# prime-slam/octreelib

Hardware: NVIDIA B200
Metric: points/sec (insert+subdivide+per-leaf RANSAC) (higher is better)
Workload: dtype f64

## Files before the change

octreelib_b200/csrc/common.cuh:

```cuda
#pragma once
#include <cuda_runtime.h>
#include <math.h>
#include <stdint.h>
#include <stdio.h>
#include <stdlib.h>
#include <string.h>

#include <algorithm>
#include <iterator>
#include <map>
#include <mutex>
#include <string>
#include <vector>

#include "../../include/octreelib_b200.h"

namespace ol {

struct Error {
    int code;
    std::string msg;
};

void set_last_error(int code, const std::string& msg);
// ... 316 lines not shown
    void raw_free(void* p) {
        if (g_block_cache.put(cache_key(), p)) return;
        if (free_fn)
            free_fn(alloc_user, p);
        else
            cudaFreeAsync(p, stream);
    }
    void sync() { OL_CUDA(cudaStreamSynchronize(stream)); }

    static constexpr size_t STATUS_POOL_WORDS = (size_t)1 << 20;
    unsigned long long* status_pool = nullptr;
    size_t status_used = 0;
    unsigned long long* status_words(size_t words) {
        words = (words + 1) & ~(size_t)1;
        if (status_used + words > STATUS_POOL_WORDS) return nullptr;
        if (!status_pool) {
            status_pool = static_cast<unsigned long long*>(alloc(STATUS_POOL_WORDS * 8));
            OL_CUDA(cudaMemsetAsync(status_pool, 0, STATUS_POOL_WORDS * 8, stream));
        }
        unsigned long long* p = status_pool + status_used;
        status_used += words;
        return p;
    }
    ~Ctx() {
        if (status_pool) free(status_pool, STATUS_POOL_WORDS * 8);
        trim_pool();
        release_arena();
    }
};

struct PoolScope {
    Ctx& c;
    explicit PoolScope(Ctx& ctx) : c(ctx) { c.pool_enabled = true; }
    ~PoolScope() {
        c.pool_enabled = false;
        c.trim_pool();
    }
};

struct ProfScope {
    Ctx& c;
    Profiler::Rec rec{};
    bool on;
    ProfScope(Ctx& ctx, const char* name, double units = 0.0) : c(ctx), on(ctx.prof && ctx.prof->enabled) {
        if (on) {
            rec.name = name;
            rec.units = units;
            rec.a = c.prof->get_event();
            rec.b = c.prof->get_event();
            cudaEventRecord(rec.a, c.stream);
        }
    }
    ~ProfScope() {
        if (on) {
            cudaEventRecord(rec.b, c.stream);
            c.prof->recs.push_back(rec);
        }
    }
};

struct Mail {
    volatile unsigned long long* slot = nullptr;
    unsigned long long ticket = 0;
    const uint32_t* err = nullptr;
    const uint32_t* aux = nullptr;
};
struct MailResult {
    unsigned long long total = 0;
    uint32_t err = 0, aux = 0;
};
#ifdef __CUDACC__
__device__ __forceinline__ void mail_post(const Mail& m, unsigned long long total) {
    if (!m.slot) return;
    m.slot[1] = total;
    m.slot[2] = m.err ? (unsigned long long)*reinterpret_cast<const volatile uint32_t*>(m.err) : 0ull;
    m.slot[3] = m.aux ? (unsigned long long)*reinterpret_cast<const volatile uint32_t*>(m.aux) : 0ull;
    __threadfence_system();
    m.slot[0] = m.ticket;
}
#endif
extern unsigned long long g_mail_ticket;
MailResult mail_wait(const Mail& m, cudaStream_t stream);

template <typename T>
struct DevBuf {
    Ctx* ctx = nullptr;
    T* ptr = nullptr;
    size_t count = 0;

    DevBuf() = default;
    DevBuf(Ctx& c, size_t n) { reset(c, n); }
    DevBuf(const DevBuf&) = delete;
    DevBuf& operator=(const DevBuf&) = delete;
    DevBuf(DevBuf&& o) noexcept { *this = std::move(o); }
    DevBuf& operator=(DevBuf&& o) noexcept {
        if (this != &o) {
            release();
            ctx = o.ctx;
            ptr = o.ptr;
            count = o.count;
            o.ptr = nullptr;
            o.count = 0;
        }
        return *this;
    }
    ~DevBuf() { release(); }
    void reset(Ctx& c, size_t n) {
        release();
        ctx = &c;
        count = n;
        ptr = static_cast<T*>(c.alloc(n * sizeof(T)));
    }
    void release() {
        if (ptr && ctx) ctx->free(ptr, count * sizeof(T));
        ptr = nullptr;
        count = 0;
    }
    void swap(DevBuf& o) {
        std::swap(ctx, o.ctx);
        std::swap(ptr, o.ptr);
        std::swap(count, o.count);
    }
    void zero() {
        if (count) OL_CUDA(cudaMemsetAsync(ptr, 0, count * sizeof(T), ctx->stream));
    }
    T* get() const { return ptr; }
    size_t size() const { return count; }
};

template <typename T>
inline void d2h(Ctx& c, T* host, const T* dev, size_t n) {
    if (n) OL_CUDA(cudaMemcpyAsync(host, dev, n * sizeof(T), cudaMemcpyDeviceToHost, c.stream));
}
template <typename T>
inline void h2d(Ctx& c, T* dev, const T* host, size_t n) {
    if (n) OL_CUDA(cudaMemcpyAsync(dev, host, n * sizeof(T), cudaMemcpyHostToDevice, c.stream));
}
template <typename T>
inline void d2d(Ctx& c, T* dst, const T* src, size_t n) {
    if (n) OL_CUDA(cudaMemcpyAsync(dst, src, n * sizeof(T), cudaMemcpyDeviceToDevice, c.stream));
}

inline unsigned grid_for(size_t n, int threads) { return (unsigned)((n + threads - 1) / threads); }

__host__ __device__ inline double npy_floor_divide_ref(double a, double b) {
    if (b == 0.0) return a / b;
    double mod = fmod(a, b);
    double div = (a - mod) / b;
    if (mod != 0.0) {
        if ((b < 0) != (mod < 0)) {
            div -= 1.0;
        }
    }
    double floordiv;
    if (div != 0.0) {
        floordiv = floor(div);
        if (div - floordiv > 0.5) floordiv += 1.0;
    } else {
        floordiv = copysign(0.0, a / b);
    }
    return floordiv;
}

__host__ __device__ inline double npy_floor_divide(double a, double b) {
    if (!(b > 0.0) || !(fabs(a) < 1.7e308) || !(b < 1.7e308)) return npy_floor_divide_ref(a, b);
    double q = floor(a / b);
// ... 40 lines not shown
```

octreelib_b200/csrc/forest.cu:

```cuda
#include <algorithm>
#include <climits>
#include <exception>
#include <mutex>

#include "forest.cuh"
#include "primitives.cuh"

namespace ol {

__device__ __forceinline__ int seg_of_rank(const uint32_t* __restrict__ seg_start, int n_seg, uint32_t r) {
    const uint32_t total = seg_start[n_seg];
    int s = (int)((float)r * __fdividef((float)n_seg, (float)(total ? total : 1u)));
    s = s < 0 ? 0 : (s >= n_seg ? n_seg - 1 : s);
    int lo = 0, hi = n_seg;
#pragma unroll 1
    for (int probe = 0; probe < 3; ++probe) {
        if (seg_start[s] > r) {
            hi = s;
            s = s - 1;
        } else if (seg_start[s + 1] <= r) {
            lo = s + 1;
            s = s + 1;
        } else {
            return s;
// ... 145 lines not shown
                qa = 0.0;
            }
            q[a] = (long long)qa;
            long long rel = q[a] - kp.qmin[a];
            if (rel < 0) {
                e |= DEVERR_CELL_RANGE;
                rel = 0;
            }
            if (kp.shift[a] < 64) key |= ((uint64_t)rel) << kp.shift[a];
        }
    }
    if (kp.pose_bits) key |= (uint64_t)seg_pose[seg_of_rank(seg_start, n_seg, r)];
    double c[3];
#pragma unroll
    for (int a = 0; a < 3; ++a) c[a] = cell_corner_coord(q[a], kp.corner[a], kp.edge, kp.single_cell);
    int bad;
    MortT m = (MortT)point_morton(p, c, kp.edge, kp.depth, &bad);
    if (embed_levels > 0) {
        key = (key << (3 * embed_levels + 1)) | ((uint64_t)(bad < kp.depth ? 1u : 0u) << (3 * embed_levels)) | (uint64_t)m;
    } else {
        if (bad < kp.depth) m |= MortBits<MortT>::bad;
        mort[r] = m;
    }
    keys[r] = (KeyT)key;
    vals[r] = r;
    if (e) atomicOr(err, e);
}

template <typename MortT>
__global__ void __launch_bounds__(256) remorton_kernel(const double* __restrict__ xyz, const uint32_t* __restrict__ perm,
                                                       const uint32_t* __restrict__ cell_of, const uint32_t* __restrict__ lcell,
                                                       const uint64_t* __restrict__ cell_key, KeyParams kp, uint32_t n,
                                                       MortT* __restrict__ mort) {
    uint32_t i = blockIdx.x * blockDim.x + threadIdx.x;
    if (i >= n) return;
    const size_t r = perm[i];
    uint32_t c = cell_of[i];
    if (lcell) c = lcell[c];
    long long q[3] = {0, 0, 0};
    if (!kp.single_cell) unpack_cell(kp, cell_key[c], q);
    const double p[3] = {xyz[r * 3], xyz[r * 3 + 1], xyz[r * 3 + 2]};
    double c0[3];
#pragma unroll
    for (int a = 0; a < 3; ++a) c0[a] = cell_corner_coord(q[a], kp.corner[a], kp.edge, kp.single_cell);
    int bad;
    MortT m = (MortT)point_morton(p, c0, kp.edge, kp.depth, &bad);
    if (bad < kp.depth) m |= MortBits<MortT>::bad;
    mort[i] = m;
}

template <typename KeyT>
struct CellKeyFn {
    const KeyT* keys;
    int pose_bits;
    __device__ uint64_t operator()(uint32_t i) const { return (uint64_t)(keys[i] >> pose_bits); }
};
template <typename KeyT>
struct CellKeyEmbedFn {
    const KeyT* keys;
    int shift;
    int fw;
    uint32_t* mort_out;
    __device__ uint64_t operator()(uint32_t i) const {
        const KeyT k = keys[i];
        const uint32_t field = (uint32_t)k & ((1u << fw) - 1u);
        mort_out[i] = (field & ((1u << (fw - 1)) - 1u)) | ((field >> (fw - 1)) ? MortBits<uint32_t>::bad : 0u);
        return (uint64_t)(k >> shift);
    }
};
struct CellEmitFn {
    uint64_t* cell_key;
    uint32_t* cell_start;
    __device__ void operator()(uint32_t run, uint32_t i, uint64_t key) const {
        cell_key[run] = key;
        cell_start[run] = i;
    }
};
struct GroupPoseKeyFn {
    const uint32_t* group;
    const uint32_t* perm;
    const uint32_t* seg_start;
    const int32_t* seg_pose;
    int n_seg;
    __device__ uint64_t operator()(uint32_t i) const {
        return ((uint64_t)group[i] << 32) | (uint64_t)(uint32_t)seg_pose[seg_of_rank(seg_start, n_seg, perm[i])];
    }
};
struct CellPoseEmitFn {
    uint32_t* cp_cell;
    int32_t* cp_pose;
    int32_t* cell_first_pose;
    const uint32_t* cellidx;
    __device__ void operator()(uint32_t run, uint32_t i, uint64_t key) const {
        const uint32_t cell = (uint32_t)(key >> 32);
        cp_cell[run] = cell;
        cp_pose[run] = (int32_t)(uint32_t)key;
        if (i == 0 || cellidx[i - 1] != cell) cell_first_pose[cell] = (int32_t)(uint32_t)key;
    }
};
struct BlockEmitFn {
    uint32_t* blk_start;
    uint32_t* blk_leaf;
    int32_t* blk_pose;
    __device__ void operator()(uint32_t run, uint32_t i, uint64_t key) const {
        blk_start[run] = i;
        blk_leaf[run] = (uint32_t)(key >> 32);
        blk_pose[run] = (int32_t)(uint32_t)key;
    }
};

constexpr int CMP_THREADS = 256;
constexpr int CMP_TILE = 2048;
constexpr int CMP_WORDS = CMP_TILE / 32;

__global__ void __launch_bounds__(CMP_THREADS) keep_bits_kernel(const uint8_t* __restrict__ keep, const uint32_t* __restrict__ via,
                                                                uint32_t n, uint32_t* __restrict__ bits,
                                                                uint32_t* __restrict__ tile_cnt) {
    __shared__ uint32_t s_cnt;
    if (threadIdx.x == 0) s_cnt = 0;
    __syncthreads();
    const uint32_t base = blockIdx.x * CMP_TILE;
    const int lane = threadIdx.x & 31;
    uint32_t c = 0;
    uint8_t flag[CMP_TILE / CMP_THREADS];
#pragma unroll
    for (int j = 0; j < CMP_TILE / CMP_THREADS; ++j) {
        const uint32_t i = base + j * CMP_THREADS + threadIdx.x;
        flag[j] = i < n ? keep[via ? via[i] : i] : (uint8_t)0;
    }
#pragma unroll
    for (int j = 0; j < CMP_TILE / CMP_THREADS; ++j) {
        const uint32_t i = base + j * CMP_THREADS + threadIdx.x;
        const bool k = flag[j] != 0;
        const uint32_t m = __ballot_sync(0xffffffffu, k);
        if (lane == 0 && i < n) {
            bits[i >> 5] = m;
            c += __popc(m);
        }
    }
    if (lane == 0 && c) atomicAdd(&s_cnt, c);
    __syncthreads();
    if (threadIdx.x == 0) tile_cnt[blockIdx.x] = s_cnt;
}

template <typename MortT>
__global__ void __launch_bounds__(CMP_THREADS) compact_move_kernel(const uint32_t* __restrict__ bits, const uint32_t* __restrict__ tile_off,
                                                                   uint32_t n, const uint32_t* __restrict__ perm_in,
                                                                   const MortT* __restrict__ mort_in, const uint32_t* __restrict__ aux_in,
                                                                   uint32_t* __restrict__ perm_out, MortT* __restrict__ mort_out,
                                                                   uint32_t* __restrict__ aux_out, uint32_t* __restrict__ word_off) {
    __shared__ uint32_t s_mask[CMP_WORDS], s_off[CMP_WORDS], s_half;
    const uint32_t base = blockIdx.x * CMP_TILE;
    const uint32_t n_words = (n + 31) >> 5;
    const int lane = threadIdx.x & 31, warp = threadIdx.x >> 5;
    if (threadIdx.x < CMP_WORDS) {
        const uint32_t w = (base >> 5) + threadIdx.x;
        const uint32_t m = w < n_words ? bits[w] : 0u;
        const uint32_t c = __popc(m);
        uint32_t inc = c;
#pragma unroll
        for (int d = 1; d < 32; d <<= 1) {
            const uint32_t v = __shfl_up_sync(0xffffffffu, inc, d);
            if (lane >= d) inc += v;
        }
        if (threadIdx.x == 31) s_half = inc;
        s_mask[threadIdx.x] = m;
        s_off[threadIdx.x] = inc - c;
    }
    __syncthreads();
// ... 548 lines not shown
__global__ void cell_first_leaf_kernel(uint32_t L, const uint32_t* __restrict__ lcell, uint32_t* __restrict__ cell_leaf_begin) {
    uint32_t k = blockIdx.x * blockDim.x + threadIdx.x;
    if (k >= L) return;
    const uint32_t c = lcell[k];
    if (k == 0 || lcell[k - 1] != c) cell_leaf_begin[c] = k;
}

__global__ void leaf_order_geometry_kernel(uint32_t L, const uint32_t* __restrict__ lcell, const int32_t* __restrict__ lparent,
                                           const uint8_t* __restrict__ lchild, const uint64_t* __restrict__ lpath,
                                           const uint8_t* __restrict__ ldepth, const uint32_t* __restrict__ irank,
                                           const uint32_t* __restrict__ imask, const uint32_t* __restrict__ leafbase,
                                           const uint32_t* __restrict__ cell_ifirst, const uint32_t* __restrict__ cell_leaf_begin,
                                           const uint64_t* __restrict__ cell_key, KeyParams kp, uint32_t* __restrict__ cache_rank,
                                           uint32_t* __restrict__ leaf_by_cache, double* __restrict__ corner,
                                           double* __restrict__ edge) {
    uint32_t k = blockIdx.x * blockDim.x + threadIdx.x;
    if (k >= L) return;
    const uint32_t c = lcell[k];
    uint32_t j = cell_leaf_begin[c];
    const int32_t p = lparent[k];
    if (p >= 0) {
        const uint32_t ch = lchild[k];
        j += leafbase[irank[p]] - leafbase[cell_ifirst[c]] + (uint32_t)__popc(~imask[p] & ((1u << ch) - 1u));
    }
    cache_rank[k] = j;
    leaf_by_cache[j] = k;
    long long q[3] = {0, 0, 0};
    if (!kp.single_cell) unpack_cell(kp, cell_key[c], q);
    double co[3];
    for (int a = 0; a < 3; ++a) co[a] = cell_corner_coord(q[a], kp.corner[a], kp.edge, kp.single_cell);
    double e = kp.edge;
    const int depth = ldepth[k];
    const uint64_t path = lpath[k];
    for (int d = 0; d < depth; ++d) {
        const double h = e * 0.5;
        const uint32_t dig = (uint32_t)(path >> (3 * (depth - 1 - d))) & 7u;
        if (dig & 4u) co[0] = co[0] + h;
        if (dig & 2u) co[1] = co[1] + h;
        if (dig & 1u) co[2] = co[2] + h;
        e = h;
    }
    corner[(size_t)j * 3 + 0] = co[0];
    corner[(size_t)j * 3 + 1] = co[1];
    corner[(size_t)j * 3 + 2] = co[2];
    edge[j] = e;
}

__global__ void __launch_bounds__(256) block_max_kernel(const uint32_t* __restrict__ blk_start, const unsigned long long* __restrict__ d_nb,
                                                        uint32_t* __restrict__ out_max) {
    __shared__ uint32_t s_w[8];
    const uint32_t nb = (uint32_t)*d_nb;
    uint32_t v = 0;
    for (uint32_t b = blockIdx.x * blockDim.x + threadIdx.x; b < nb; b += gridDim.x * blockDim.x) {
        const uint32_t sz = blk_start[b + 1] - blk_start[b];
        v = sz > v ? sz : v;
    }
#pragma unroll
    for (int o = 16; o > 0; o >>= 1) {
        uint32_t t = __shfl_xor_sync(0xffffffffu, v, o);
        v = t > v ? t : v;
    }
    if ((threadIdx.x & 31) == 0) s_w[threadIdx.x >> 5] = v;
    __syncthreads();
    if (threadIdx.x == 0) {
        for (int w = 1; w < 8; ++w) v = s_w[w] > v ? s_w[w] : v;
        if (v) atomicMax(out_max, v);
    }
}

__global__ void block_keep_kernel(uint32_t nb, const uint32_t* __restrict__ blk_start, const int32_t* __restrict__ blk_pose,
                                  const uint8_t* __restrict__ listed, const uint8_t* __restrict__ table,
                                  long long table_len, uint8_t* __restrict__ keep_blk) {
    uint32_t b = blockIdx.x * blockDim.x + threadIdx.x;
    if (b >= nb) return;
    uint8_t keep = 1;
    if (!listed || listed[blk_pose[b]]) {
        long long sz = (long long)(blk_start[b + 1] - blk_start[b]);
        if (sz > table_len - 1) sz = table_len - 1;
        keep = table[sz];
    }
    keep_blk[b] = keep;
}

__global__ void pos_keep_from_block_kernel(uint32_t n, const uint32_t* __restrict__ blk_of_pos,
                                           const uint8_t* __restrict__ keep_blk, uint8_t* __restrict__ keep_pos) {
    uint32_t i = blockIdx.x * blockDim.x + threadIdx.x;
    if (i < n) keep_pos[i] = keep_blk[blk_of_pos[i]];
}

}

#include "forest_host.inl"
#include "forest_host2.inl"
```

octreelib_b200/csrc/forest.cuh:

```cuda
#pragma once
#include <initializer_list>
#include <vector>

#include "common.cuh"
#include "pointkey.cuh"

namespace ol {

constexpr int MORTON_INITIAL_DEPTH = 8;
constexpr int MORTON32_MAX_DEPTH = 10;

struct Forest {
    Ctx ctx;
    ol_forest_config cfg{};
    int max_depth = OL_MAX_DEPTH;

    DevBuf<double> P64;
    size_t cap = 0, N = 0;
    size_t bbox_done = 0;
    bool q_known = false;
    long long q_lo[3] = {0, 0, 0}, q_hi[3] = {0, 0, 0};
    bool points_external() const { return P64.ptr != nullptr && P64.ctx == nullptr; }
    void adopt_points(double* ext, size_t n, const int64_t* seg_sizes, const int32_t* seg_pose_in, const int64_t* seg_first_in,
                      int n_segments, int n_poses_total, const long long qlo[3], const long long qhi[3]);
// ... 25 lines not shown
    bool cells_pending = false, blocks_pending = false;
    Mail cells_mail{}, blocks_mail{};
    DevBuf<unsigned long long> d_nb;
    void resolve_cells();
    void resolve_blocks();
    void resolve_pending() {
        resolve_cells();
        resolve_blocks();
    }
    void build_enqueue();
    void ensure_blocks_enqueue();
    void prefetch_tables();

    bool built = false;
    KeyParams kp{};
    int key_bits = 0;
    int key_embed = 0;
    uint32_t A0 = 0;
    DevBuf<uint32_t> perm0;
    DevBuf<uint64_t> mort0;
    bool mort32 = true;
    size_t mort_len(size_t n) const { return mort32 ? (n + 1) / 2 : n; }
    DevBuf<uint32_t> cellidx0;
    uint32_t C = 0;
    DevBuf<uint64_t> cell_key;
    DevBuf<uint32_t> cell_start0;
    uint32_t CP = 0;
    bool cp_valid = false;
    DevBuf<uint32_t> cp_cell;
    DevBuf<int32_t> cp_pose;
    DevBuf<int32_t> cell_first_pose;

    bool shaped = false;
    bool order_virgin = false;
    uint32_t A = 0;
    uint32_t A_shape = 0;
    DevBuf<uint32_t> perm;
    DevBuf<uint64_t> mort;
    DevBuf<uint32_t> leaf_of;
    uint32_t L = 0;
    DevBuf<uint32_t> lstart;
    DevBuf<uint32_t> lcell;
    DevBuf<int32_t> lparent;
    DevBuf<uint64_t> lpath;
    DevBuf<uint8_t> ldepth;
    DevBuf<uint8_t> lchild;
    uint32_t I = 0;
    size_t icap = 0;
    DevBuf<uint32_t> istart;
    DevBuf<uint32_t> icell;
    DevBuf<uint8_t> idepth;
    DevBuf<uint64_t> ipath;
    DevBuf<int32_t> iparent;
    DevBuf<uint8_t> ichild;
    std::vector<uint32_t> level_ibegin;
    int depth_reached = 0;

    bool order_valid = false;
    DevBuf<uint32_t> cache_rank;
    DevBuf<uint32_t> leaf_by_cache;
    DevBuf<double> leaf_corner;
    DevBuf<double> leaf_edge;
    DevBuf<uint32_t> cell_leaf_begin;

    bool replay_pending = false;
    uint32_t sp_n = 0;
    DevBuf<long long> sp_q;
    DevBuf<uint32_t> sp_depth;
    DevBuf<uint64_t> sp_path;
    DevBuf<uint32_t> sp_epoch;

    int n_subdivide_calls = 0;
    std::vector<int> pose_epoch;
    bool epochs_valid = false;
    DevBuf<uint32_t> iepoch;
    bool history_active() const { return n_subdivide_calls >= 2 && epochs_valid && I > 0; }
    void assign_epochs(int epoch, const uint64_t* sorted_keys, const uint32_t* sorted_vals, uint32_t n_saved);

    bool blocks_valid = false;
    uint32_t NB = 0;
    DevBuf<uint32_t> blk_start;
    DevBuf<uint32_t> blk_leaf;
    DevBuf<int32_t> blk_pose;
    DevBuf<uint32_t> blk_of_pos;
    uint32_t max_block = 0;
    bool max_block_known = false;
    bool max_block_enqueued = false;
    void enqueue_max_block();
    DevBuf<uint32_t> d_max_block;

    bool ransac_valid = false;
    DevBuf<uint8_t> mask;
    uint32_t mask_n = 0;
    uint32_t res_n = 0;
    DevBuf<int32_t> res_pose, res_leaf, res_size, res_best, res_count;
    DevBuf<float> res_plane;
    bool snap_pending = false;
    DevBuf<uint32_t> sn_ref_order, sn_leaf;
    DevBuf<uint32_t> sn_arr_rank, sn_arr_blk;
    int sn_rank_bits = 0;
    int sn_K = 0;
    DevBuf<int32_t> sn_pose, sn_size, sn_best, sn_count;
    DevBuf<float> sn_plane;
    bool sample_oob_seen = false;
    uint32_t last_ransac_work = 0;
    Profiler prof;

    explicit Forest(const ol_forest_config& c);
    ~Forest();

    int insert(const double* xyz, int64_t n, bool on_device, const int64_t* seg_sizes, const int32_t* seg_pose_in,
               const int64_t* seg_first_in, int n_segments, int n_poses_total);
    int insert_batch(const double* const* xyz_dev, const int64_t* sizes, int count);
    void build();
    void ensure_cell_poses();
    void compact_base();
    struct CompactTables {
        DevBuf<uint32_t> bits, word_off, tile_off;
    };
    uint32_t compact_tables(const uint8_t* keep, const uint32_t* via, uint32_t n, CompactTables& t);
    void compact_move(CompactTables& t, uint32_t n, const uint32_t* perm_in, const uint64_t* mort_in, const uint32_t* aux_in,
                      uint32_t* perm_out, uint64_t* mort_out, uint32_t* aux_out);
    void ensure_alive();
    void extend_morton();
    void reset_shape();
    struct SplitRule {
        std::vector<int> first_level;
        std::vector<int64_t> max_points;
        const uint8_t* tables_host = nullptr;
        int64_t table_len = 0;
        std::vector<int> beyond;
        std::vector<ol_geom_term> terms;
        std::vector<int> term_begin;
        int n_terms(int e) const { return term_begin.empty() ? 0 : term_begin[e + 1] - term_begin[e]; }
        bool needs_cov(int e) const {
            for (int t = 0; t < n_terms(e); ++t)
                if (terms[term_begin[e] + t].stat == OL_GEOM_THICKNESS) return true;
            return false;
        }
        int64_t geom_min_points(int e) const {
            int64_t m = INT64_MAX;
            for (int t = 0; t < n_terms(e); ++t) {
                const ol_geom_term& g = terms[term_begin[e] + t];
                m = std::min<int64_t>(m, g.op == OL_GEOM_GT ? std::max<int64_t>(g.min_points, 1) : g.min_points);
            }
            return m;
        }
        int entry_for(int level) const {
            int e = 0;
            for (size_t i = 0; i < first_level.size(); ++i)
                if (first_level[i] <= level) e = (int)i;
            return e;
        }
    };
    void subdivide(const SplitRule& rule, const int32_t* poses, int n_poses_listed);
    void split_levels(const SplitRule* rule, const uint8_t* d_tables, const uint8_t* d_listed, int n_listed,
                      const uint64_t* replay_keys, uint32_t n_replay, const ol_geom_term* d_terms = nullptr);
    void reserve_internal(size_t need);
    void ensure_max_block();
    struct ReadItem {
        const void* src;
        size_t bytes;
        void* dst;
    };
    void read_back(std::initializer_list<ReadItem> items);
    void throw_device_errors(uint32_t e);
    void note_ransac_flags(uint32_t e);
// ... 48 lines not shown
```

octreelib_b200/csrc/primitives.cuh:

```cuda
#pragma once
#include "common.cuh"
#include "onesweep.cuh"

namespace ol {

constexpr int SCAN_THREADS = 256;
constexpr size_t SCAN_SMALL_MAX = 16384;
constexpr unsigned long long SCAN_VALID = 1ull << 63;

__device__ __forceinline__ uint32_t warp_inclusive_scan(uint32_t v) {
#pragma unroll
    for (int o = 1; o < 32; o <<= 1) {
        uint32_t t = __shfl_up_sync(0xffffffffu, v, o);
        if ((threadIdx.x & 31) >= o) v += t;
    }
    return v;
}
__device__ __forceinline__ unsigned long long warp_inclusive_scan64(unsigned long long v) {
#pragma unroll
    for (int o = 1; o < 32; o <<= 1) {
        unsigned long long t = __shfl_up_sync(0xffffffffu, v, o);
        if ((threadIdx.x & 31) >= o) v += t;
    }
    return v;
}

__device__ __forceinline__ uint32_t block_exclusive_scan_256(uint32_t v, uint32_t* smem_warp , uint32_t* total) {
    const int lane = threadIdx.x & 31, warp = threadIdx.x >> 5;
    uint32_t inc = warp_inclusive_scan(v);
    if (lane == 31) smem_warp[warp] = inc;
    __syncthreads();
    uint32_t wsum = (lane < 8) ? smem_warp[lane] : 0;
    uint32_t winc = warp_inclusive_scan(wsum);
    uint32_t wbase = __shfl_sync(0xffffffffu, winc - wsum, warp);
    uint32_t tot = __shfl_sync(0xffffffffu, winc, 7);
    __syncthreads();
    if (total) *total = tot;
    return wbase + inc - v;
}

__device__ __forceinline__ unsigned long long block_exclusive_scan64(unsigned long long v, unsigned long long* smem_warp ,
                                                                    unsigned long long* total) {
    const int lane = threadIdx.x & 31, warp = threadIdx.x >> 5, nwarps = blockDim.x >> 5;
    unsigned long long inc = warp_inclusive_scan64(v);
    if (lane == 31) smem_warp[warp] = inc;
    __syncthreads();
    unsigned long long wsum = (lane < nwarps) ? smem_warp[lane] : 0ull;
    unsigned long long winc = warp_inclusive_scan64(wsum);
    unsigned long long wbase = __shfl_sync(0xffffffffu, winc - wsum, warp);
    unsigned long long tot = __shfl_sync(0xffffffffu, winc, nwarps - 1);
    __syncthreads();
    if (total) *total = tot;
    return wbase + inc - v;
}

__device__ __forceinline__ unsigned long long scan_ld_status(const unsigned long long* p) {
    unsigned long long v;
    asm volatile("ld.relaxed.gpu.global.u64 %0, [%1];" : "=l"(v) : "l"(p) : "memory");
    return v;
}
__device__ __forceinline__ void scan_st_status(unsigned long long* p, unsigned long long v) {
    asm volatile("st.relaxed.gpu.global.u64 [%0], %1;" ::"l"(p), "l"(v) : "memory");
}
__device__ __forceinline__ void scan_ld_status2(const unsigned long long* p, unsigned long long& agg, unsigned long long& inc) {
    asm volatile("ld.relaxed.gpu.global.v2.u64 {%0, %1}, [%2];" : "=l"(agg), "=l"(inc) : "l"(p) : "memory");
}
__device__ __forceinline__ unsigned long long lookback_exclusive_prefix(unsigned long long* __restrict__ status, uint32_t tile,
                                                                        unsigned long long aggregate,
                                                                        unsigned long long* s_prefix ) {
    (void)s_prefix;
    __shared__ unsigned long long s_sum[32];
    __shared__ uint32_t s_stop[32];
    const int lane = threadIdx.x & 31, warp = threadIdx.x >> 5, nwarps = (int)(blockDim.x >> 5);
    if (threadIdx.x == 0) scan_st_status(status + 2 * (size_t)tile + (tile == 0 ? 1 : 0), SCAN_VALID | aggregate);
    unsigned long long prefix = 0;
    if (tile > 0) {
        long long look = (long long)tile - 1;
        while (true) {
            const long long idx = look - (long long)threadIdx.x;
            unsigned long long val = 0;
            bool stop = idx < 0;
            if (idx >= 0) {
                while (true) {
                    unsigned long long agg, inc;
                    scan_ld_status2(status + 2 * (size_t)idx, agg, inc);
// ... 216 lines not shown
#pragma unroll
    for (int j = 0; j < SORT_ITEMS; ++j) {
        uint32_t i = wbase + j * 32 + lane;
        bool valid = i < n;
        k[j] = valid ? keys_in[i] : (KeyT)0;
        uint32_t d = valid ? (uint32_t)((k[j] >> shift) & mask) : 0xffffffffu;
        uint32_t peers = __match_any_sync(0xffffffffu, d);
        int leader = __ffs(peers) - 1;
        uint32_t old = 0;
        if (valid && lane == leader) {
            old = whist[warp][d];
            whist[warp][d] = old + __popc(peers);
        }
        old = __shfl_sync(0xffffffffu, old, leader);
        rnk[j] = old + __popc(peers & lt);
        __syncwarp();
    }
    __syncthreads();
    for (uint32_t b = threadIdx.x; b < nbins; b += SORT_THREADS) {
        uint32_t run = offsets[(size_t)b * num_tiles + blockIdx.x];
#pragma unroll
        for (int w = 0; w < SORT_WARPS; ++w) {
            uint32_t t = whist[w][b];
            whist[w][b] = run;
            run += t;
        }
    }
    __syncthreads();
#pragma unroll
    for (int j = 0; j < SORT_ITEMS; ++j) {
        uint32_t i = wbase + j * 32 + lane;
        if (i < n) {
            uint32_t d = (uint32_t)((k[j] >> shift) & mask);
            uint32_t dst = whist[warp][d] + rnk[j];
            keys_out[dst] = k[j];
            vals_out[dst] = vals_in[i];
        }
    }
}

extern bool g_force_legacy_sort;
template <typename KeyT>
inline int radix_sort_pairs(Ctx& c, KeyT* keys0, KeyT* keys1, uint32_t* vals0, uint32_t* vals1, size_t n, int begin_bit,
                            int end_bit, bool main_sort = false) {
    OL_REQUIRE(n < (1ull << 31), OL_ERR_INVALID, "radix_sort_pairs: n must be < 2^31");
    int bits = end_bit - begin_bit;
    if (n <= 1 || bits <= 0) return 0;
    if (n < (1ull << 30) && !g_force_legacy_sort) return onesweep_sort_pairs<KeyT>(c, keys0, keys1, vals0, vals1, n, begin_bit, end_bit, main_sort);
    int passes = (bits + 7) / 8;
    int per = (bits + passes - 1) / passes;
    uint32_t tiles = (uint32_t)((n + SORT_TILE - 1) / SORT_TILE);
    DevBuf<uint32_t> counts(c, (size_t)256 * tiles);
    int cur = 0;
    int bit = begin_bit;
    for (int p = 0; p < passes; ++p) {
        int nb = (end_bit - bit < per) ? (end_bit - bit) : per;
        uint32_t nbins = 1u << nb;
        KeyT* kin = cur ? keys1 : keys0;
        KeyT* kout = cur ? keys0 : keys1;
        uint32_t* vin = cur ? vals1 : vals0;
        uint32_t* vout = cur ? vals0 : vals1;
        {
            ProfScope ps(c, sizeof(KeyT) == 8 ? "radix_hist_u64" : "radix_hist_u32", (double)n);
            radix_hist_kernel<KeyT><<<tiles, SORT_THREADS, 0, c.stream>>>(kin, counts.get(), (uint32_t)n, tiles, bit, nbins);
            OL_CHECK_LAUNCH();
        }
        exclusive_scan_u32(c, counts.get(), counts.get(), (size_t)nbins * tiles, nullptr);
        {
            ProfScope ps(c, sizeof(KeyT) == 8 ? "radix_scatter_u64" : "radix_scatter_u32", (double)n);
            radix_scatter_kernel<KeyT><<<tiles, SORT_THREADS, 0, c.stream>>>(kin, vin, kout, vout, counts.get(), (uint32_t)n,
                                                                               tiles, bit, nbins);
            OL_CHECK_LAUNCH();
        }
        cur ^= 1;
        bit += nb;
    }
    return cur;
}

constexpr int RUNS_THREADS = 256;
constexpr int RUNS_ITEMS = 8;
constexpr int RUNS_TILE = RUNS_THREADS * RUNS_ITEMS;

template <typename KeyFn>
__device__ __forceinline__ void runs_warp_flags(const KeyFn& key, uint32_t wbase, uint32_t n, int lane, uint32_t masks[RUNS_ITEMS],
                                                uint64_t keys[RUNS_ITEMS]) {
    uint64_t carry = 0;
    bool have_carry = false;
    if (wbase > 0 && wbase < n) {
        carry = key(wbase - 1);
        have_carry = true;
    }
#pragma unroll
    for (int j = 0; j < RUNS_ITEMS; ++j) {
        const uint32_t i = wbase + 32 * j + lane;
        keys[j] = i < n ? key(i) : 0ull;
    }
#pragma unroll
    for (int j = 0; j < RUNS_ITEMS; ++j) {
        const uint32_t i = wbase + 32 * j + lane;
        const bool valid = i < n;
        const uint64_t k = keys[j];
        uint64_t prev = __shfl_up_sync(0xffffffffu, k, 1);
        bool has_prev = true;
        if (lane == 0) {
            prev = carry;
            has_prev = have_carry;
        }
        const bool head = valid && (!has_prev || prev != k);
        masks[j] = __ballot_sync(0xffffffffu, head);
        carry = __shfl_sync(0xffffffffu, k, 31);
        have_carry = true;
    }
}

template <typename KeyFn, typename EmitFn>
__global__ void __launch_bounds__(RUNS_THREADS) runs_fused_kernel(KeyFn key, EmitFn emit, uint32_t n, uint32_t num_tiles,
                                                                  unsigned long long* __restrict__ status,
                                                                  uint32_t* __restrict__ run_of_pos,
                                                                  unsigned long long* __restrict__ total_out,
                                                                  uint32_t* __restrict__ sentinel, const Mail mail) {
    __shared__ uint32_t s_w[RUNS_THREADS / 32];
    __shared__ unsigned long long s_prefix;
    __shared__ uint32_t s_tile;
    if (threadIdx.x == 0) s_tile = atomicAdd(reinterpret_cast<uint32_t*>(status + 2 * (size_t)num_tiles), 1u);
    __syncthreads();
    const uint32_t tile = s_tile;
    const int lane = threadIdx.x & 31, warp = threadIdx.x >> 5;
    const uint32_t wbase = tile * RUNS_TILE + warp * (32 * RUNS_ITEMS);
    uint32_t masks[RUNS_ITEMS];
    uint64_t keys[RUNS_ITEMS];
    runs_warp_flags(key, wbase, n, lane, masks, keys);
    uint32_t cnt = 0;
#pragma unroll
    for (int j = 0; j < RUNS_ITEMS; ++j) cnt += __popc(masks[j]);
    if (lane == 0) s_w[warp] = cnt;
    __syncthreads();
    uint32_t tile_total = 0, before = 0;
#pragma unroll
    for (int w = 0; w < RUNS_THREADS / 32; ++w) {
        if (w < warp) before += s_w[w];
        tile_total += s_w[w];
    }
    const unsigned long long prefix = lookback_exclusive_prefix(status, tile, (unsigned long long)tile_total, &s_prefix);
    if (tile == num_tiles - 1 && threadIdx.x == 0) {
        if (total_out) *total_out = prefix + tile_total;
        if (sentinel) sentinel[prefix + tile_total] = n;
        mail_post(mail, prefix + tile_total);
    }
    uint32_t run = (uint32_t)prefix + before;
    const uint32_t lt = (1u << lane) - 1u;
#pragma unroll
    for (int j = 0; j < RUNS_ITEMS; ++j) {
        const uint32_t i = wbase + 32 * j + lane;
        const bool head = (masks[j] >> lane) & 1u;
        const uint32_t mine = run + __popc(masks[j] & lt) + (head ? 1u : 0u) - 1u;
        if (i < n) {
            if (run_of_pos) run_of_pos[i] = mine;
            if (head) emit(mine, i, keys[j]);
        }
        run += __popc(masks[j]);
    }
}

template <typename KeyFn>
__global__ void __launch_bounds__(RUNS_THREADS) runs_flags_kernel(KeyFn key, uint32_t n, uint32_t* __restrict__ flag_words,
                                                                  uint32_t* __restrict__ tile_cnt) {
    __shared__ uint32_t s_w[RUNS_THREADS / 32];
    const uint32_t tile = blockIdx.x;
    const int lane = threadIdx.x & 31, warp = threadIdx.x >> 5;
    const uint32_t wbase = tile * RUNS_TILE + warp * (32 * RUNS_ITEMS);
    uint32_t masks[RUNS_ITEMS];
    uint64_t keys[RUNS_ITEMS];
    runs_warp_flags(key, wbase, n, lane, masks, keys);
    uint32_t cnt = 0;
#pragma unroll
    for (int j = 0; j < RUNS_ITEMS; ++j) {
        cnt += __popc(masks[j]);
        if (lane == j && wbase + 32 * j < n) flag_words[(wbase >> 5) + j] = masks[j];
    }
    if (lane == 0) s_w[warp] = cnt;
    __syncthreads();
    if (threadIdx.x == 0) {
        uint32_t t = 0;
#pragma unroll
        for (int w = 0; w < RUNS_THREADS / 32; ++w) t += s_w[w];
        tile_cnt[tile] = t;
    }
}

template <typename KeyFn, typename EmitFn>
__global__ void __launch_bounds__(RUNS_THREADS) runs_emit2_kernel(KeyFn key, EmitFn emit, uint32_t n, uint32_t num_tiles,
                                                                  const uint32_t* __restrict__ flag_words,
                                                                  const uint32_t* __restrict__ tile_off,
                                                                  const unsigned long long* __restrict__ d_total,
                                                                  uint32_t* __restrict__ run_of_pos, uint32_t* __restrict__ sentinel) {
    __shared__ uint32_t s_w[RUNS_THREADS / 32];
    const uint32_t tile = blockIdx.x;
    const int lane = threadIdx.x & 31, warp = threadIdx.x >> 5;
    const uint32_t wbase = tile * RUNS_TILE + warp * (32 * RUNS_ITEMS);
    uint32_t masks[RUNS_ITEMS];
    uint32_t cnt = 0;
#pragma unroll
    for (int j = 0; j < RUNS_ITEMS; ++j) {
        masks[j] = wbase + 32 * j < n ? flag_words[(wbase >> 5) + j] : 0u;
        cnt += __popc(masks[j]);
    }
    if (lane == 0) s_w[warp] = cnt;
    __syncthreads();
    uint32_t run = tile_off[tile];
#pragma unroll
    for (int w = 0; w < RUNS_THREADS / 32; ++w)
        if (w < warp) run += s_w[w];
    const uint32_t lt = (1u << lane) - 1u;
#pragma unroll
    for (int j = 0; j < RUNS_ITEMS; ++j) {
        const uint32_t i = wbase + 32 * j + lane;
        const bool head = (masks[j] >> lane) & 1u;
        const uint32_t mine = run + __popc(masks[j] & lt) + (head ? 1u : 0u) - 1u;
        if (i < n) {
            if (run_of_pos) run_of_pos[i] = mine;
            if (head) emit(mine, i, key(i));
        }
        run += __popc(masks[j]);
    }
    if (tile == num_tiles - 1 && threadIdx.x == 0 && sentinel) sentinel[*d_total] = n;
}
constexpr size_t RUNS_TWO_PASS_MIN = (size_t)1 << 20;

template <typename KeyFn, typename EmitFn>
inline void segment_runs(Ctx& c, KeyFn key, EmitFn emit, size_t n, uint32_t* run_of_pos, unsigned long long* d_total,
                         uint32_t* sentinel = nullptr, const Mail& mail = Mail{}) {
    OL_REQUIRE(n > 0, OL_ERR_INTERNAL, "segment_runs: empty input");
    const size_t tiles = (n + RUNS_TILE - 1) / RUNS_TILE;
    static const bool one_pass = getenv("OL_RUNS_ONE_PASS") != nullptr;
    if (n >= RUNS_TWO_PASS_MIN && !one_pass) {
        OL_REQUIRE(d_total != nullptr, OL_ERR_INTERNAL, "segment_runs: the two-pass form needs a device total");
        DevBuf<uint32_t> flag_words(c, (n + 31) / 32), tile_cnt(c, tiles);
        runs_flags_kernel<KeyFn><<<(unsigned)tiles, RUNS_THREADS, 0, c.stream>>>(key, (uint32_t)n, flag_words.get(), tile_cnt.get());
        OL_CHECK_LAUNCH();
        transform_scan<uint32_t>(c, ScanPtrIn<uint32_t>{tile_cnt.get()}, ScanPtrOut<uint32_t>{tile_cnt.get()}, tiles, d_total, "scan", mail);
        runs_emit2_kernel<KeyFn, EmitFn><<<(unsigned)tiles, RUNS_THREADS, 0, c.stream>>>(key, emit, (uint32_t)n, (uint32_t)tiles,
                                                                                         flag_words.get(), tile_cnt.get(), d_total,
                                                                                         run_of_pos, sentinel);
        OL_CHECK_LAUNCH();
        return;
    }
    DevBuf<unsigned long long> own;
    unsigned long long* status = c.status_words(2 * tiles + 1);
    if (!status) {
        own.reset(c, 2 * tiles + 1);
        own.zero();
        status = own.get();
    }
    runs_fused_kernel<KeyFn, EmitFn><<<(unsigned)tiles, RUNS_THREADS, 0, c.stream>>>(key, emit, (uint32_t)n, (uint32_t)tiles, status,
                                                                                     run_of_pos, d_total, sentinel, mail);
    OL_CHECK_LAUNCH();
}

static __global__ void iota_kernel(uint32_t* out, uint32_t n, uint32_t first) {
    uint32_t i = blockIdx.x * blockDim.x + threadIdx.x;
    if (i < n) out[i] = first + i;
}

template <typename T>
__global__ void fill_kernel(T* out, size_t n, T v) {
    size_t i = (size_t)blockIdx.x * blockDim.x + threadIdx.x;
    if (i < n) out[i] = v;
}

template <typename T>
__global__ void gather_kernel(T* __restrict__ out, const T* __restrict__ in, const uint32_t* __restrict__ idx, size_t n) {
    size_t i = (size_t)blockIdx.x * blockDim.x + threadIdx.x;
    if (i < n) out[i] = in[idx[i]];
}

inline int bit_length_u64(uint64_t v) {
    int b = 0;
    while (v) {
        ++b;
        v >>= 1;
    }
    return b;
}

}
```

Baseline: 8.041 billion.

## Replace materialized blk_of_pos with bitmask run index and split key load/finish

Segment runs can now keep the head-flag bit words and a per-word run offset. A RunIndex then answers run-of-position queries with a popcount instead of a full per-point blk_of_pos array, which is built only on demand through a lazy ensure path. Key functors get a split load/finish so the global loads for all items are issued before the dependent segment-rank lookup, and the emit pass reloads keys only for run heads. The host-side wiring (ensure_blk_of_pos, blk_words allocation) is not shown, so whether the blocks path actually uses the index is uncertain.

```diff
diff --git a/octreelib_b200/csrc/common.cuh b/octreelib_b200/csrc/common.cuh
--- a/octreelib_b200/csrc/common.cuh
+++ b/octreelib_b200/csrc/common.cuh
@@ -422,6 +422,19 @@
 extern unsigned long long g_mail_ticket;
 MailResult mail_wait(const Mail& m, cudaStream_t stream);
 
+#ifdef __CUDACC__
+struct RunIndex {
+    const uint32_t* words;
+    const uint32_t* word_off;
+    const unsigned long long* d_total;
+    uint32_t n;
+    __device__ __forceinline__ uint32_t runs_before(uint32_t p) const {
+        if (p >= n) return (uint32_t)*d_total;
+        return word_off[p >> 5] + __popc(words[p >> 5] & ((1u << (p & 31)) - 1u));
+    }
+};
+#endif
+
 template <typename T>
 struct DevBuf {
     Ctx* ctx = nullptr;
diff --git a/octreelib_b200/csrc/forest.cu b/octreelib_b200/csrc/forest.cu
--- a/octreelib_b200/csrc/forest.cu
+++ b/octreelib_b200/csrc/forest.cu
@@ -251,9 +251,11 @@
     const uint32_t* seg_start;
     const int32_t* seg_pose;
     int n_seg;
-    __device__ uint64_t operator()(uint32_t i) const {
-        return ((uint64_t)group[i] << 32) | (uint64_t)(uint32_t)seg_pose[seg_of_rank(seg_start, n_seg, perm[i])];
-    }
+    __device__ __forceinline__ uint64_t load(uint32_t i) const { return ((uint64_t)group[i] << 32) | (uint64_t)perm[i]; }
+    __device__ __forceinline__ uint64_t finish(uint64_t v) const {
+        return (v & 0xffffffff00000000ull) | (uint64_t)(uint32_t)seg_pose[seg_of_rank(seg_start, n_seg, (uint32_t)v)];
+    }
+    __device__ uint64_t operator()(uint32_t i) const { return finish(load(i)); }
 };
 struct CellPoseEmitFn {
     uint32_t* cp_cell;
@@ -968,6 +970,11 @@
     keep_blk[b] = keep;
 }
 
+__global__ void run_of_pos_kernel(RunIndex ri, uint32_t n, uint32_t* __restrict__ run_of_pos) {
+    const uint32_t i = blockIdx.x * blockDim.x + threadIdx.x;
+    if (i < n) run_of_pos[i] = ri.runs_before(i + 1) - 1u;
+}
+
 __global__ void pos_keep_from_block_kernel(uint32_t n, const uint32_t* __restrict__ blk_of_pos,
                                            const uint8_t* __restrict__ keep_blk, uint8_t* __restrict__ keep_pos) {
     uint32_t i = blockIdx.x * blockDim.x + threadIdx.x;
diff --git a/octreelib_b200/csrc/forest.cuh b/octreelib_b200/csrc/forest.cuh
--- a/octreelib_b200/csrc/forest.cuh
+++ b/octreelib_b200/csrc/forest.cuh
@@ -131,7 +131,12 @@
     DevBuf<uint32_t> blk_start;
     DevBuf<uint32_t> blk_leaf;
     DevBuf<int32_t> blk_pose;
+    DevBuf<uint32_t> blk_words;
+    DevBuf<uint32_t> blk_word_off;
+    RunIndex blk_index() const { return RunIndex{blk_words.get(), blk_word_off.get(), d_nb.get(), A}; }
     DevBuf<uint32_t> blk_of_pos;
+    bool blk_of_pos_valid = false;
+    void ensure_blk_of_pos();
     uint32_t max_block = 0;
     bool max_block_known = false;
     bool max_block_enqueued = false;
diff --git a/octreelib_b200/csrc/primitives.cuh b/octreelib_b200/csrc/primitives.cuh
--- a/octreelib_b200/csrc/primitives.cuh
+++ b/octreelib_b200/csrc/primitives.cuh
@@ -1,6 +1,8 @@
 #pragma once
 #include "common.cuh"
 #include "onesweep.cuh"
+
+#include <type_traits>
 
 namespace ol {
 
@@ -383,6 +385,17 @@
 constexpr int RUNS_ITEMS = 8;
 constexpr int RUNS_TILE = RUNS_THREADS * RUNS_ITEMS;
 
+template <typename KeyFn, typename = void>
+struct RunKey {
+    static __device__ __forceinline__ uint64_t load(const KeyFn& k, uint32_t i) { return k(i); }
+    static __device__ __forceinline__ uint64_t finish(const KeyFn&, uint64_t v) { return v; }
+};
+template <typename KeyFn>
+struct RunKey<KeyFn, std::void_t<decltype(&KeyFn::finish)>> {
+    static __device__ __forceinline__ uint64_t load(const KeyFn& k, uint32_t i) { return k.load(i); }
+    static __device__ __forceinline__ uint64_t finish(const KeyFn& k, uint64_t v) { return k.finish(v); }
+};
+
 template <typename KeyFn>
 __device__ __forceinline__ void runs_warp_flags(const KeyFn& key, uint32_t wbase, uint32_t n, int lane, uint32_t masks[RUNS_ITEMS],
                                                 uint64_t keys[RUNS_ITEMS]) {
@@ -395,8 +408,11 @@
 #pragma unroll
     for (int j = 0; j < RUNS_ITEMS; ++j) {
         const uint32_t i = wbase + 32 * j + lane;
-        keys[j] = i < n ? key(i) : 0ull;
-    }
+        keys[j] = i < n ? RunKey<KeyFn>::load(key, i) : 0ull;
+    }
+#pragma unroll
+    for (int j = 0; j < RUNS_ITEMS; ++j)
+        if (wbase + 32 * j + lane < n) keys[j] = RunKey<KeyFn>::finish(key, keys[j]);
 #pragma unroll
     for (int j = 0; j < RUNS_ITEMS; ++j) {
         const uint32_t i = wbase + 32 * j + lane;
@@ -495,7 +511,8 @@
                                                                   const uint32_t* __restrict__ flag_words,
                                                                   const uint32_t* __restrict__ tile_off,
                                                                   const unsigned long long* __restrict__ d_total,
-                                                                  uint32_t* __restrict__ run_of_pos, uint32_t* __restrict__ sentinel) {
+                                                                  uint32_t* __restrict__ run_of_pos, uint32_t* __restrict__ sentinel,
+                                                                  uint32_t* __restrict__ word_off) {
     __shared__ uint32_t s_w[RUNS_THREADS / 32];
     const uint32_t tile = blockIdx.x;
     const int lane = threadIdx.x & 31, warp = threadIdx.x >> 5;
@@ -514,14 +531,21 @@
     for (int w = 0; w < RUNS_THREADS / 32; ++w)
         if (w < warp) run += s_w[w];
     const uint32_t lt = (1u << lane) - 1u;
+    uint64_t loaded[RUNS_ITEMS];
+#pragma unroll
+    for (int j = 0; j < RUNS_ITEMS; ++j) {
+        const uint32_t i = wbase + 32 * j + lane;
+        loaded[j] = i < n && ((masks[j] >> lane) & 1u) ? RunKey<KeyFn>::load(key, i) : 0ull;
+    }
 #pragma unroll
     for (int j = 0; j < RUNS_ITEMS; ++j) {
         const uint32_t i = wbase + 32 * j + lane;
         const bool head = (masks[j] >> lane) & 1u;
         const uint32_t mine = run + __popc(masks[j] & lt) + (head ? 1u : 0u) - 1u;
+        if (word_off && lane == j && wbase + 32 * j < n) word_off[(wbase >> 5) + j] = run;
         if (i < n) {
             if (run_of_pos) run_of_pos[i] = mine;
-            if (head) emit(mine, i, key(i));
+            if (head) emit(mine, i, RunKey<KeyFn>::finish(key, loaded[j]));
         }
         run += __popc(masks[j]);
     }
@@ -531,19 +555,24 @@
 
 template <typename KeyFn, typename EmitFn>
 inline void segment_runs(Ctx& c, KeyFn key, EmitFn emit, size_t n, uint32_t* run_of_pos, unsigned long long* d_total,
-                         uint32_t* sentinel = nullptr, const Mail& mail = Mail{}) {
+                         uint32_t* sentinel = nullptr, const Mail& mail = Mail{}, uint32_t* words = nullptr,
+                         uint32_t* word_off = nullptr) {
     OL_REQUIRE(n > 0, OL_ERR_INTERNAL, "segment_runs: empty input");
     const size_t tiles = (n + RUNS_TILE - 1) / RUNS_TILE;
     static const bool one_pass = getenv("OL_RUNS_ONE_PASS") != nullptr;
-    if (n >= RUNS_TWO_PASS_MIN && !one_pass) {
+    if ((n >= RUNS_TWO_PASS_MIN && !one_pass) || words) {
         OL_REQUIRE(d_total != nullptr, OL_ERR_INTERNAL, "segment_runs: the two-pass form needs a device total");
-        DevBuf<uint32_t> flag_words(c, (n + 31) / 32), tile_cnt(c, tiles);
-        runs_flags_kernel<KeyFn><<<(unsigned)tiles, RUNS_THREADS, 0, c.stream>>>(key, (uint32_t)n, flag_words.get(), tile_cnt.get());
+        DevBuf<uint32_t> own_words, tile_cnt(c, tiles);
+        if (!words) {
+            own_words.reset(c, (n + 31) / 32);
+            words = own_words.get();
+        }
+        runs_flags_kernel<KeyFn><<<(unsigned)tiles, RUNS_THREADS, 0, c.stream>>>(key, (uint32_t)n, words, tile_cnt.get());
         OL_CHECK_LAUNCH();
         transform_scan<uint32_t>(c, ScanPtrIn<uint32_t>{tile_cnt.get()}, ScanPtrOut<uint32_t>{tile_cnt.get()}, tiles, d_total, "scan", mail);
         runs_emit2_kernel<KeyFn, EmitFn><<<(unsigned)tiles, RUNS_THREADS, 0, c.stream>>>(key, emit, (uint32_t)n, (uint32_t)tiles,
-                                                                                         flag_words.get(), tile_cnt.get(), d_total,
-                                                                                         run_of_pos, sentinel);
+                                                                                         words, tile_cnt.get(), d_total,
+                                                                                         run_of_pos, sentinel, word_off);
         OL_CHECK_LAUNCH();
         return;
     }
```

Result: faster. 8.317 billion (median of 6 runs) (+3.4%).
